# nuclia/nucliadb

Hardware: AMD Instinct MI355X
Metric: queries/sec + recall@10 (768-dim cosine k-NN, HNSW M=30 ef=30 ef_upper=4 build_ef_upper=4, k=10) (higher is better)
Workload: dtype f32

## Files before the change

### include/nidx_gpu.h

```cpp
#ifndef NIDX_GPU_H
#define NIDX_GPU_H

#include <stddef.h>
#include <stdint.h>

#ifdef __cplusplus
extern "C" {
#endif

#define NIDX_OK 0
#define NIDX_ERR_IO (-1)
#define NIDX_ERR_INCONSISTENT_DIMENSIONS (-2)
#define NIDX_ERR_INVALID_CONFIGURATION (-3)
#define NIDX_ERR_EMPTY_MERGE (-4)
#define NIDX_ERR_INVALID_ARGUMENT (-5)
#define NIDX_ERR_UNSUPPORTED (-6)
#define NIDX_ERR_DEVICE (-7)
#define NIDX_ERR_INVALID_GRAPH (-8)
#define NIDX_ERR_INEXACT (-9)
#define NIDX_ERR_OUT_OF_MEMORY (-10)
#define NIDX_ERR_INTERNAL (-11)
#define NIDX_ERR_BUSY (-12)

int32_t nidx_gpu_last_error(char *buf, size_t len);
// ... 244 lines not shown

int32_t nidx_gpu_similarity(const float *x, const float *y, uint32_t n_pairs, uint32_t dimension,
                            int32_t similarity, int32_t order, float *out);
int32_t nidx_gpu_normalize(const float *in, uint32_t n, uint32_t dimension, float *out);

int32_t nidx_gpu_hnsw_graph_check(const uint8_t *graph, uint64_t graph_len, const float *edges, uint64_t n_edges, uint32_t n_nodes,
                                  uint32_t *entry_node_out, uint32_t *entry_layer_out, uint64_t *n_links_out,
                                  uint64_t *n_broken_links_out);

int32_t nidx_gpu_vector_build_hnsw(nidx_gpu_vector_index_t *index, uint32_t segment, uint64_t level_seed);
int32_t nidx_gpu_vector_build_stats(nidx_gpu_vector_index_t *index, uint64_t *stats_out);
int32_t nidx_gpu_vector_extend_hnsw(nidx_gpu_vector_index_t *index, uint32_t segment, uint64_t level_seed);
int32_t nidx_gpu_vector_serialize_hnsw(const nidx_gpu_vector_index_t *index, uint32_t segment, uint8_t *graph_out,
                                       uint64_t graph_cap, uint64_t *graph_len_out, float *edges_out,
                                       uint64_t edges_cap, uint64_t *n_edges_out);

typedef struct nidx_gpu_segment_dir nidx_gpu_segment_dir_t;
int32_t nidx_gpu_segment_dir_open(const char *path, uint32_t dimension, nidx_gpu_segment_dir_t **dir_out);
void nidx_gpu_segment_dir_close(nidx_gpu_segment_dir_t *dir);
int32_t nidx_gpu_segment_dir_index_source(const nidx_gpu_segment_dir_t *dir);
int32_t nidx_gpu_segment_dir_segment(const nidx_gpu_segment_dir_t *dir, nidx_gpu_vector_segment_t *segment_out);
int32_t nidx_gpu_segment_dir_filter_index(const nidx_gpu_segment_dir_t *dir, nidx_gpu_filter_index_t *lists_out);
enum { NIDX_LIST_LABEL = 0, NIDX_LIST_FIELD = 1 };
int32_t nidx_gpu_segment_dir_lists(const nidx_gpu_segment_dir_t *dir, int32_t kind, const uint8_t *key, uint32_t key_len,
                                   int32_t prefix, uint32_t *first_out, uint32_t *count_out);
typedef struct {
    const char *key;
    uint32_t key_len;
    const uint8_t *metadata;
    uint32_t metadata_len;
// ... 615 lines not shown
```

### nucliadb_amd/_lib.py

```python
from __future__ import annotations

import ctypes as C
import os

_HERE = os.path.dirname(os.path.abspath(__file__))
LIB_PATH = os.environ.get("NIDX_GPU_LIB") or os.path.join(_HERE, "libnidx_gpu.so")

NIDX_OK = 0
NIDX_ERR_IO = -1
NIDX_ERR_INCONSISTENT_DIMENSIONS = -2
NIDX_ERR_INVALID_CONFIGURATION = -3
NIDX_ERR_EMPTY_MERGE = -4
NIDX_ERR_INVALID_ARGUMENT = -5
NIDX_ERR_UNSUPPORTED = -6
NIDX_ERR_DEVICE = -7
NIDX_ERR_INVALID_GRAPH = -8
NIDX_ERR_INEXACT = -9
NIDX_ERR_OUT_OF_MEMORY = -10
NIDX_ERR_INTERNAL = -11
NIDX_ERR_BUSY = -12

SIMILARITY_DOT, SIMILARITY_COSINE = 0, 1
METHOD_AUTO, METHOD_HNSW, METHOD_BRUTE_FORCE, METHOD_BRUTE_FORCE_MFMA, METHOD_BRUTE_FORCE_BF16 = 0, 1, 2, 3, 4
METHOD_RABITQ_HNSW, METHOD_RABITQ_BRUTE_FORCE = 5, 6
# ... 430 lines not shown
                                                C.c_void_p, C.c_void_p, C.c_void_p, C.c_void_p]),
    "nidx_gpu_vector_search_maxsim_filtered_per_query": (C.c_int32, [C.c_void_p, C.c_void_p, C.c_void_p, C.c_uint32, C.c_uint32,
                                                                     C.POINTER(VectorSearchParamsC), C.c_void_p, C.c_uint32, C.c_void_p,
                                                                     C.c_void_p, C.c_void_p, C.c_void_p, C.c_void_p]),
    "nidx_gpu_vector_search_maxsim_submit": (C.c_int32, [C.c_void_p, C.c_void_p, C.c_void_p, C.c_uint32, C.c_uint32,
                                                         C.POINTER(VectorSearchParamsC), C.c_void_p, C.POINTER(C.c_uint64)]),
    "nidx_gpu_vector_search_maxsim_submit_filtered_per_query": (C.c_int32, [C.c_void_p, C.c_void_p, C.c_void_p, C.c_uint32, C.c_uint32,
                                                                            C.POINTER(VectorSearchParamsC), C.c_void_p, C.c_uint32,
                                                                            C.c_void_p, C.POINTER(C.c_uint64)]),
    "nidx_gpu_vector_search_maxsim_wait": (C.c_int32, [C.c_void_p, C.c_uint64, C.c_void_p, C.c_void_p, C.c_void_p, C.c_void_p]),
    "nidx_gpu_vector_maxsim_stats": (C.c_int32, [C.c_void_p, C.POINTER(C.c_uint64), C.POINTER(C.c_uint64)]),
    "nidx_gpu_vector_quantize": (C.c_int32, [C.c_void_p, C.c_uint32]),
    "nidx_gpu_vector_serialize_quantized": (C.c_int32, [C.c_void_p, C.c_uint32, C.c_void_p, C.c_uint64, C.POINTER(C.c_uint64)]),
    "nidx_gpu_vector_serialize_hnsw": (C.c_int32, [C.c_void_p, C.c_uint32, C.c_void_p, C.c_uint64, C.POINTER(C.c_uint64),
                                                   C.c_void_p, C.c_uint64, C.POINTER(C.c_uint64)]),
    "nidx_gpu_bm25_open": (C.c_int32, [C.POINTER(Bm25SegmentC), C.c_uint32, C.POINTER(C.c_void_p)]),
    "nidx_gpu_bm25_close": (None, [C.c_void_p]),
    "nidx_gpu_bm25_space_usage": (C.c_int32, [C.c_void_p, C.POINTER(C.c_uint64)]),
    "nidx_gpu_bm25_search": (C.c_int32, [C.c_void_p, C.c_void_p, C.c_void_p, C.c_uint32, C.c_uint32, C.c_void_p, C.c_void_p,
                                         C.c_void_p, C.c_void_p, C.c_void_p, C.c_void_p]),
    "nidx_gpu_bm25_search_ex": (C.c_int32, [C.c_void_p, C.c_void_p, C.c_void_p, C.c_uint32, C.POINTER(Bm25SearchOptionsC), C.c_void_p,
                                          C.c_void_p, C.c_void_p, C.c_void_p, C.c_void_p]),
    "nidx_gpu_bm25_search_submit": (C.c_int32, [C.c_void_p, C.c_void_p, C.c_void_p, C.c_uint32, C.POINTER(Bm25SearchOptionsC), C.POINTER(C.c_uint64)]),
    "nidx_gpu_bm25_search_wait": (C.c_int32, [C.c_void_p, C.c_uint64, C.c_void_p, C.c_void_p, C.c_void_p, C.c_void_p, C.c_void_p]),
    "nidx_gpu_bm25_set_fast_field": (C.c_int32, [C.c_void_p, C.c_uint32, C.c_uint32, C.c_void_p]),
    "nidx_gpu_bm25_set_dictionary": (C.c_int32, [C.c_void_p, C.c_void_p, C.c_void_p]),
    "nidx_gpu_bm25_sync": (C.c_int32, [C.c_void_p, C.POINTER(Bm25SyncEntryC), C.c_uint32, C.c_uint32, C.c_void_p, C.c_void_p, C.c_void_p, C.c_uint32,
                                       C.c_void_p, C.c_void_p, C.POINTER(Bm25SyncStatsC)]),
    "nidx_gpu_bm25_generation": (C.c_int32, [C.c_void_p, C.POINTER(C.c_uint64)]),
    "nidx_gpu_segment_dir_open": (C.c_int32, [C.c_char_p, C.c_uint32, C.POINTER(C.c_void_p)]),
# ... 173 lines not shown
```

### nucliadb_amd/csrc/hnsw_build.hip

```cpp
#include <stdlib.h>

#include <hipcub/hipcub.hpp>

#include "hnsw_device.h"
#include "hnsw_graph.h"

namespace nidx {

struct BuildArgs {
    SegDev seg;
    GraphDev g;
    float *l0_w;
    float *upper_w;
    const uint8_t *levels;
    uint32_t batch_start, batch_size;
    const uint32_t *slot_base;
    uint64_t *found;
    uint32_t *found_len;
    uint32_t *slot_node;
    uint32_t *slot_layer;
    uint64_t *req_key;
    float *req_val;
    uint32_t vis_log2;
    uint32_t ef_upper;
// ... 328 lines not shown
    e = hipcub::DeviceRadixSort::SortPairs(sort_tmp, sort_tmp_bytes, a.req_key, req_key_sorted, a.req_val,
                                           req_val_sorted, (int)n_req, 0, 64, s);
    if (e != hipSuccess) return e;
    if (minw == 4) hipLaunchKernelGGL((reverse_link_kernel<NJ, 4>), dim3((n_req + 3) / 4), dim3(256), 0, s, a, req_key_sorted, req_val_sorted, n_req);
    else if (minw == 2) hipLaunchKernelGGL((reverse_link_kernel<NJ, 2>), dim3((n_req + 3) / 4), dim3(256), 0, s, a, req_key_sorted, req_val_sorted, n_req);
    else hipLaunchKernelGGL((reverse_link_kernel<NJ, 3>), dim3((n_req + 3) / 4), dim3(256), 0, s, a, req_key_sorted, req_val_sorted, n_req);
    return hipGetLastError();
}

__global__ void flag_clear_kernel(uint32_t *word, uint32_t bits) { atomicAnd(word, ~bits); }
hipError_t launch_flag_clear(uint32_t *word, uint32_t bits, hipStream_t s) {
    hipLaunchKernelGGL(flag_clear_kernel, dim3(1), dim3(1), 0, s, word, bits);
    return hipGetLastError();
}

hipError_t build_sort_tmp_bytes(uint32_t max_req, size_t *bytes) {
    *bytes = 0;
    return hipcub::DeviceRadixSort::SortPairs(nullptr, *bytes, (uint64_t *)nullptr, (uint64_t *)nullptr,
                                              (float *)nullptr, (float *)nullptr, (int)max_req, 0, 64, nullptr);
}

hipError_t launch_build_batch(const BuildBatch &b, hipStream_t s) {
    BuildArgs a;
    a.seg = b.seg;
    a.g = b.g;
    a.l0_w = b.l0_w;
    a.upper_w = b.upper_w;
    a.levels = b.levels;
    a.batch_start = b.batch_start;
    a.batch_size = b.batch_size;
// ... 29 lines not shown
```

### nucliadb_amd/csrc/hnsw_build_host.cpp

```cpp
#include <stdlib.h>

#include <algorithm>
#include <chrono>

#include "host_common.h"
#include "vector_index.h"

namespace nidx {

static const uint32_t kMaxBatch = 32768;

int32_t VectorIndex::build_hnsw(uint32_t si, uint64_t level_seed, bool extend) {
    std::lock_guard<std::mutex> lock(mu);
    NIDX_HIP(hipSetDevice(device));
    VectorSegment &seg = segs[si];
    const uint32_t n = seg.n;
    if (extend && !seg.base_graph) return fail(NIDX_ERR_INVALID_ARGUMENT, "segment %u was not opened with a partial hnsw graph", si);
    const uint32_t n0 = extend ? seg.base_nodes : 0;
    const HostGraph *base = extend ? seg.base_graph.get() : nullptr;
    seg.has_graph = false;
    if (n == 0) return NIDX_OK;
    if (n >= (1u << 30)) return fail(NIDX_ERR_UNSUPPORTED, "segments of 2^30 or more vectors are not supported");
    std::vector<uint8_t> drawn, levels(n);
    draw_levels(level_seed, n - n0, drawn);
// ... 179 lines not shown
                d5[1] ? d5[2] / d5[1] : 0, d5[3] ? (double)d5[2] / (double)d5[3] : 0.0);
    }
    if (flags & NIDX_FLAG_POOL_INEXACT) return fail(NIDX_ERR_INEXACT, "HNSW build: candidate pool overflow");
    last_build_flags = flags;
    {
        std::vector<unsigned long long> lines((size_t)NIDX_BUILD_STAT_LINES * 16, 0ull);
        if (b.stats) NIDX_HIP(hipMemcpy(lines.data(), b.stats, lines.size() * 8, hipMemcpyDeviceToHost));
        for (int c = 0; c < 8; c++) last_build_stats[c] = 0;
        for (size_t l = 0; l < NIDX_BUILD_STAT_LINES; l++)
            for (int c = 0; c < 6; c++) last_build_stats[2 + c] += lines[l * 16 + c];
        last_build_stats[0] = n - n0;
        last_build_stats[1] = (uint64_t)std::chrono::duration<double, std::micro>(std::chrono::steady_clock::now() - t_build0).count();
        if (!b.stats) last_build_stats[2] = ~0ull;
    }
    seg.has_graph = true;
    seg.base_graph.reset();
    seg.base_nodes = 0;
    return NIDX_OK;
}

}

using namespace nidx;

extern "C" int32_t nidx_gpu_vector_build_hnsw(nidx_gpu_vector_index_t *index, uint32_t segment, uint64_t level_seed) try {
    VectorIndex *idx = reinterpret_cast<VectorIndex *>(index);
    if (!idx) return fail(NIDX_ERR_INVALID_ARGUMENT, "bad index/segment");
    GenShared gen(idx->gate);
    if (segment >= idx->segs.size()) return fail(NIDX_ERR_INVALID_ARGUMENT, "bad index/segment");
    return idx->build_hnsw(segment, level_seed, false);
// ... 20 lines not shown
```

### nucliadb_amd/csrc/hnsw_device.h

```cpp
#pragma once
#include "device_common.h"
#include "kernels.h"

namespace nidx {

#define NIDX_POOL_CAP 512
#define NIDX_VIS_EMPTY 0xffffffffu
#define NIDX_DEFER_CAP 256

struct NbBuf {
    uint32_t addr[64];
    float ab[64];
    float xx[64];
};
struct SearchShared {
    uint64_t pool[NIDX_POOL_CAP];
    NbBuf nb[2];
    uint32_t eps[256];
    int ctrl[12];
};

template <int NJ>
struct QueryRegs {
    float4 qv[NJ];
// ... 93 lines not shown
        unsigned long long m = __ballot(keep);
        int pos = out + __popcll(m & ((1ull << lane) - 1ull));
        if (keep) pool[pos] = v;
        out += __popcll(m);
    }
    pool_len = out;
}

template <int NL>
struct CandSet {
    uint64_t unexp[NL];
    __device__ inline void init() {
#pragma unroll
        for (int i = 0; i < NL; i++) unexp[i] = 0;
    }
    __device__ inline void insert(WaveTopK<NL> &res, uint64_t nk, int cap, int lane, uint64_t &out_key, bool &out_unexp) {
        uint64_t d = nk, dflag = 1;
#pragma unroll
        for (int i = 0; i < NL; i++) {
            if (d != NIDX_EMPTY_KEY) {
                const int pos = __popcll(__ballot(res.l[i].key > d));
                if (pos < 64) {
                    const uint64_t last = lane_bcast_u64(res.l[i].key, 63);
                    const uint64_t lastflag = unexp[i] >> 63;
                    const uint64_t up = wave_shr1_u64(res.l[i].key);
                    if (lane > pos) res.l[i].key = up;
                    if (lane == pos) res.l[i].key = d;
                    const uint64_t low = unexp[i] & ((1ull << pos) - 1ull);
                    const uint64_t high = pos < 63 ? ((unexp[i] >> pos) << (pos + 1)) : 0ull;
                    unexp[i] = low | (dflag << pos) | high;
                    d = last;
                    dflag = lastflag;
                }
            }
        }
        res.len++;
        out_key = NIDX_EMPTY_KEY;
// ... 158 lines not shown
    for (;;) {
        lds_barrier();
        const int cmd = __builtin_amdgcn_readfirstlane(sh.ctrl[0]);
        const int op = cmd & 3;
        if (op == NIDX_CMD_EVAL) eval_neighbours_dynamic<NJ, EVR>(seg, q, sh.nb[(cmd >> 2) & 1], cmd >> 3, cosine, &sh.ctrl[3]);
        else if (op == NIDX_CMD_CLEAR) vis_clear(vis, vis_cap);
        lds_barrier();
        if (op == NIDX_CMD_EXIT) return;
    }
}

#define NIDX_PARK_SLOTS 4
#define NIDX_EPS_BARE 0
#define NIDX_EPS_PARKED 1
#define NIDX_EPS_CARRIED 2
template <int NJ, int EFL, int EVR, bool SPLIT = false>
__device__ inline void layer_search_block(const SegDev &seg, const GraphDev &g, int layer, int k,
                                          const QueryRegs<NJ> &q, SearchShared &sh, uint32_t *vis, uint32_t vis_log2,
                                          WaveTopK<EFL> &res, SearchCounters &st, int ep_mode = NIDX_EPS_BARE) {
    const int lane = threadIdx.x & 63;
    const bool ctl = SPLIT ? true : (nidx_tid() >> 6) == 0;
    const bool cosine = seg.similarity == 1;
    const uint32_t vis_cap = 1u << vis_log2;
    const bool carried = ep_mode == NIDX_EPS_CARRIED;
    int pool_len = 0;
    uint32_t vis_count = 0;

    if constexpr (SPLIT) {
        split_post(sh, NIDX_CMD_CLEAR, 0, 0, lane);
        vis_clear(vis, vis_cap);
        split_close();
    } else {
        vis_clear(vis, vis_cap);
        __syncthreads();
    }
    int n_new = sh.ctrl[2];
// ... 3 lines not shown
    const int n_eps = carried ? 0 : n_new;
    uint32_t ptag = 0xffffffffu, pbase = 0xffffffffu;
    uint32_t pt0 = 0xffffffffu, pt1 = 0xffffffffu, pt2 = 0xffffffffu, pt3 = 0xffffffffu;
    int n_park = 0;
    if (ep_mode != NIDX_EPS_BARE && n_new <= 64) n_park = n_new < NIDX_PARK_SLOTS ? n_new : NIDX_PARK_SLOTS;
    if (carried && ctl) {
#pragma unroll
        for (int i = 0; i < EFL; i++) {
            const int left = res.len - 64 * i;
            cand.unexp[i] = left >= 64 ? ~0ull : (left > 0 ? (1ull << left) - 1ull : 0ull);
            if (lane < left) vis_insert(vis, vis_log2, rank_key_addr(res.mine(i)));
        }
        st.evals += n_new;
        vis_count += n_new;
        if (lane < n_park) ptag = rank_key_addr(res.mine(0));
    }
    if (ctl && !carried) {
        res.init();
        if (lane < n_new) {
            uint32_t ep = sh.eps[lane];
            vis_insert(vis, vis_log2, ep);
            sh.nb[0].addr[lane] = ep;
            if (lane < n_park) ptag = ep;
        }
    }
    if (layer >= 1 && ptag != 0xffffffffu) pbase = g.upper_base[ptag];
    int ep_done = 0;
    while (ep_done < n_eps) {
        int chunk = n_eps - ep_done < 64 ? n_eps - ep_done : 64;
        if (ctl && ep_done > 0 && lane < chunk) {
            uint32_t ep = sh.eps[ep_done + lane];
            vis_insert(vis, vis_log2, ep);
            sh.nb[0].addr[lane] = ep;
        }
        if constexpr (SPLIT) {
            split_post(sh, NIDX_CMD_EVAL, 0, chunk, lane);
            split_close();
        } else {
            __syncthreads();
            eval_neighbours<NJ, EVR>(seg, q, sh.nb[0], chunk, cosine);
            __syncthreads();
        }
        if (ctl) {
            float s = lane < chunk ? score_from_sums(sh.nb[0].ab[lane], sh.nb[0].xx[lane], q.qq, q.sqrt_qq, cosine) : 0.f;
            uint32_t addr = sh.nb[0].addr[lane];
            for (int j = 0; j < chunk; j++) {
                uint64_t ek;
                bool eu;
                cand.insert(res, rank_key(lane_bcast_f32(s, j), lane_bcast_u32(addr, j)), 64 * EFL, lane, ek, eu);
            }
            st.evals += chunk;
            vis_count += chunk;
        }
        ep_done += chunk;
    }
    if (ctl && n_park > 0) {
        pt0 = lane_bcast_u32(ptag, 0);
        pt1 = lane_bcast_u32(ptag, 1);
        pt2 = lane_bcast_u32(ptag, 2);
        pt3 = lane_bcast_u32(ptag, 3);
        uint32_t w[NIDX_PARK_SLOTS];
#pragma unroll
        for (int r = 0; r < NIDX_PARK_SLOTS; r++) {
            w[r] = 0;
            if (r < n_park) {
                const uint32_t node = lane_bcast_u32(ptag, r), b = lane_bcast_u32(pbase, r);
                if (layer == 0) w[r] = g.l0[(size_t)node * NIDX_L0_STRIDE + lane];
                else if (b != 0xffffffffu && lane < NIDX_UP_STRIDE) w[r] = g.upper[((size_t)b + (layer - 1)) * NIDX_UP_STRIDE + lane];
            }
        }
#pragma unroll
        for (int r = 0; r < NIDX_PARK_SLOTS; r++)
            if (r < n_park) sh.eps[r * 64 + lane] = w[r];
    }

    uint32_t pw0 = 0, pw1 = 0, tg0 = 0xffffffffu, tg1 = 0xffffffffu;
    uint32_t edge_hits = 0;
    auto prepare = [&](uint64_t ck, NbBuf &dst) -> int {
        uint32_t deg;
        const uint32_t node = rank_key_addr(ck);
        uint32_t w;
        const int slot = node == pt0 ? 0 : (node == pt1 ? 1 : (node == pt2 ? 2 : (node == pt3 ? 3 : -1)));
        if (slot >= 0) {
            w = sh.eps[slot * 64 + lane];
            deg = lane_bcast_u32(w, 0);
            edge_hits++;
        } else if (node == tg0) {
            w = pw0;
            deg = lane_bcast_u32(w, 0);
            edge_hits++;
        } else if (node == tg1) {
            w = pw1;
            deg = lane_bcast_u32(w, 0);
            edge_hits++;
        } else {
            w = load_edge_word(g, node, layer, lane, deg);
        }
        const bool fresh = lane >= 1 && lane <= (int)deg && !vis_contains(vis, vis_log2, w);
        const unsigned long long m = __ballot(fresh);
        if (fresh) dst.addr[__popcll(m & ((1ull << lane) - 1ull))] = w;
        return __popcll(m);
    };
    int p = 0;
    uint64_t cur = NIDX_EMPTY_KEY;
    int cont = 0, n_cur_reg = 0;
    if (ctl) {
        const uint64_t t_a = clock64();
        int n0 = 0;
        cur = cand.pop(res);
        if (cur != NIDX_EMPTY_KEY && !(rank_key_score(cur) < res.worst_score())) {
            cont = 1;
            n0 = prepare(cur, sh.nb[0]);
        }
        n_cur_reg = n0;
        if (!SPLIT && lane == 0) {
            sh.ctrl[0] = cont;
            sh.ctrl[6] = n0;
            sh.ctrl[3] = 0;
        }
        st.cyc_ctl += clock64() - t_a;
    }
    if constexpr (SPLIT) {
        if (cont) {
            split_post(sh, NIDX_CMD_EVAL, 0, n_cur_reg, lane);
            split_close();
        }
    } else {
// ... 29 lines not shown
                todo = __ballot(ins);
                const int n_valid = __popcll(todo);
                st.expansions++;
                st.evals += n_valid;
                vis_count += n_valid;
                overflow = vis_count > vis_cap - vis_cap / 4;
                s = ins ? score_from_sums(nb_cur.ab[lane], nb_cur.xx[lane], q.qq, q.sqrt_qq, cosine) : 0.f;
                int n_next = 0;
                if (!overflow) {
                    const float ws = res.worst_score();
                    const bool adm = ins && (s > ws || res.len < k);
                    const uint64_t bn = wave_max_u64(adm ? rank_key(s, addr) : NIDX_EMPTY_KEY);
                    const uint64_t pm = cand.peek(res);
                    nxt = pm > bn ? pm : bn;
                    if (nxt == NIDX_EMPTY_KEY && pool_len > 0) nxt = pool_peek(sh.pool, pool_len, lane);
                    if (nxt != NIDX_EMPTY_KEY) n_next = prepare(nxt, nb_next);
                    if (layer == 0) {
                        uint64_t ka, kb;
                        cand.peek2_except(res, nxt, ka, kb);
                        uint32_t wa = ka != NIDX_EMPTY_KEY ? rank_key_addr(ka) : 0xffffffffu;
                        uint32_t wb = kb != NIDX_EMPTY_KEY ? rank_key_addr(kb) : 0xffffffffu;
                        if (wa == tg1 || wb == tg0) {
                            const uint32_t t = wa;
                            wa = wb;
                            wb = t;
                        }
                        if (wa != tg0) {
                            tg0 = wa;
                            if (wa != 0xffffffffu) pw0 = g.l0[(size_t)wa * NIDX_L0_STRIDE + lane];
                        }
                        if (wb != tg1) {
                            tg1 = wb;
// ... 16 lines not shown
            const int n_next = SPLIT ? n_next_reg : sh.ctrl[6 + (p ^ 1)];
            if (!ctl && has_next) eval_neighbours_dynamic<NJ, EVR>(seg, q, nb_next, n_next, cosine, &sh.ctrl[3]);
            if (ctl) {
                while (todo) {
                    float ws = res.worst_score();
                    if (res.len >= k) {
                        todo &= __ballot(s > ws);
                        if (!todo) break;
                    }
                    int j = __ffsll((long long)todo) - 1;
                    todo &= ~(1ull << j);
                    float sj = lane_bcast_f32(s, j);
                    if (sj > ws || res.len < k) {
                        uint64_t ek;
                        bool eu;
                        cand.insert(res, rank_key(sj, lane_bcast_u32(addr, j)), k, lane, ek, eu);
                        if (eu && ek != NIDX_EMPTY_KEY && !(rank_key_score(ek) < res.worst_score())) {
                            if (pool_len == NIDX_POOL_CAP) {
                                pool_prune(sh.pool, pool_len, res.worst_score(), lane);
                                if (pool_len == NIDX_POOL_CAP) {
                                    st.flags |= NIDX_FLAG_POOL_INEXACT;
                                    pool_len--;
                                }
                            }
                            if (lane == 0) sh.pool[pool_len] = ek;
                            pool_len++;
                        }
                    }
                }
                int redo = 0;
                cont = 0;
// ... 14 lines not shown
                st.cyc_ins += t_c - t_b;
                if (has_next) eval_neighbours_dynamic<NJ, EVR>(seg, q, nb_next, n_next, cosine, &sh.ctrl[3]);
                st.cyc_eval += clock64() - t_c;
            }
            if constexpr (SPLIT) {
                split_close();
            } else {
                lds_barrier();
                cont = sh.ctrl[0];
                redo_reg = sh.ctrl[4];
            }
            if (!cont) break;
            n_cur_reg = n_next;
            if (redo_reg) {
                if (ctl) {
                    const int n1 = prepare(cur, nb_next);
                    n_cur_reg = n1;
                    if (!SPLIT && lane == 0) {
                        sh.ctrl[6 + (p ^ 1)] = n1;
                        sh.ctrl[3] = 0;
                    }
                }
                if constexpr (SPLIT) {
                    split_post(sh, NIDX_CMD_EVAL, p ^ 1, n_cur_reg, lane);
                    split_close();
                } else {
                    lds_barrier();
                    eval_neighbours_dynamic<NJ, EVR>(seg, q, nb_next, sh.ctrl[6 + (p ^ 1)], cosine, &sh.ctrl[3]);
                    lds_barrier();
                }
            }
// ... 9 lines not shown
```

### nucliadb_amd/csrc/hnsw_search.hip

```cpp
#include "hnsw_device.h"

namespace nidx {

template <int NJ>
__device__ inline bool rows_equal(const SegDev &seg, uint32_t a, uint32_t b, int lane) {
    const float *ra = seg.vectors + (size_t)a * seg.dp, *rb = seg.vectors + (size_t)b * seg.dp;
    bool eq = true;
#pragma unroll
    for (int j = 0; j < NJ; j++) {
        uint32_t e = (uint32_t)j * 256u + (uint32_t)lane * 4u;
        if (e < seg.dp) {
            uint4 x = *reinterpret_cast<const uint4 *>(ra + e);
            uint4 y = *reinterpret_cast<const uint4 *>(rb + e);
            eq = eq && x.x == y.x && x.y == y.y && x.z == y.z && x.w == y.w;
        }
    }
    return __all(eq);
}

template <int NJ, int EVR, int EFL, bool SPLIT>
__device__ __forceinline__ void hnsw_search_body(const HnswSearchArgs &a, const uint32_t qi, unsigned char *smem) {
    SearchShared &sh = *reinterpret_cast<SearchShared *>(smem);
    uint32_t *vis = reinterpret_cast<uint32_t *>(smem + sizeof(SearchShared));
    __shared__ uint32_t res_addr[64 * EFL];
// ... 21 lines not shown

    SearchCounters st = {0, 0, 0, 0, 0, 0, 0};
    const uint64_t t_start = clock64();
    WaveTopK<EFL> res;
    res.init();

    if (nidx_tid() == 0) {
        sh.eps[0] = a.g.ep_node;
        sh.ctrl[2] = 1;
    }
    if constexpr (!SPLIT) __syncthreads();
    const bool entry_mode = a.entry_vec != nullptr;
    const int efu = a.ef_upper ? (int)a.ef_upper : 1;
    const int top = entry_mode ? 0 : (int)a.g.ep_layer;
    for (int layer = top; layer >= 1; layer--) {
        layer_search_block<NJ, EFL, EVR, SPLIT>(a.seg, a.g, layer, efu, q, sh, vis, a.vis_log2, res, st, layer == top ? NIDX_EPS_PARKED : NIDX_EPS_CARRIED);
        if (ctl && lane == 0) sh.ctrl[2] = res.len;
    }
    const int efs = a.ef_search ? (int)a.ef_search : NIDX_EF_SEARCH;
    const int ef = k > efs ? k : efs;
    if (!entry_mode) layer_search_block<NJ, EFL, EVR, SPLIT>(a.seg, a.g, 0, ef, q, sh, vis, a.vis_log2, res, st, top >= 1 ? NIDX_EPS_CARRIED : NIDX_EPS_PARKED);
    if (a.dump_vec) {
        if (ctl) {
#pragma unroll
            for (int i = 0; i < EFL; i++) {
                const uint64_t key = res.mine(i);
                const int e = 64 * i + lane;
                if (e < res.len) {
                    a.dump_vec[(size_t)qi * NIDX_DUMP_STRIDE + e] = rank_key_addr(key);
                    a.dump_score[(size_t)qi * NIDX_DUMP_STRIDE + e] = rank_key_score(key);
                }
// ... 446 lines not shown
```

### nucliadb_amd/csrc/kernels.h

```cpp
#pragma once
#define NIDX_K_MAX 512
#include <hip/hip_runtime.h>
#include <stdint.h>

#include "../../include/nidx_gpu.h"
#include "bm25_aux_plan.h"
#include "bm25_work_plan.h"

namespace nidx {

struct ScanArgs {
    const float *vectors;
    const float *norm2;
    uint32_t n, dp;
    const float *queries;
    uint32_t n_queries;
    const uint64_t *alive;
    const uint64_t *filter;
    const uint32_t *para_of_vec;
    int similarity;
    float min_score;
    uint32_t k;
    uint32_t qt;
    uint64_t *partial;
// ... 120 lines not shown

#define NIDX_L0_STRIDE 64
#define NIDX_UP_STRIDE 32
#define NIDX_M 30
#define NIDX_M_MAX 30
#define NIDX_M_MAX0 60
#define NIDX_EF_CONSTRUCTION 100
#define NIDX_EF_SEARCH 30

struct GraphDev {
    uint32_t *l0;
    uint32_t *upper_base;
    uint32_t *upper;
    uint32_t ep_node, ep_layer;
    uint32_t n;
};

struct SegDev {
    const float *vectors;
    const float *norm2;
    uint32_t n, dp, dim;
    const uint32_t *para_of_vec;
    const uint64_t *alive;
    int similarity;
};

#define NIDX_STAT_EVALS 0
#define NIDX_STAT_EXPANSIONS 1
#define NIDX_STAT_VISITED 2
#define NIDX_STAT_FLAGS 3
#define NIDX_STAT_CYC_CTL 4
// ... 536 lines not shown
```

### nucliadb_amd/csrc/vector_index.cpp

```cpp
#include <math.h>
#include <stdio.h>
#include <stdlib.h>
#include <string.h>

#include <algorithm>
#include <unordered_map>
#include <chrono>
#include <map>
#include <memory>
#include <mutex>

#include "device_common.h"
#include "hnsw_graph.h"
#include "host_common.h"
#include "kernels.h"
#include "vector_index.h"
#include "prefilter_handover.h"

namespace nidx {

static thread_local char g_last_error[512];

static void record_error(const char *fmt, va_list ap) { vsnprintf(g_last_error, sizeof(g_last_error), fmt, ap); }

// ... 83 lines not shown
    }
    return c;
}

int32_t VectorSegment::upload_graph(const HostGraph &hg) {
    NIDX_HIP(g_l0.alloc(hg.l0.size() * 4));
    NIDX_HIP(g_upper_base.alloc(hg.upper_base.size() * 4));
    NIDX_HIP(g_upper.alloc(std::max<size_t>(hg.upper.size(), NIDX_UP_STRIDE) * 4));
    NIDX_HIP(hipMemcpy(g_l0.p, hg.l0.data(), hg.l0.size() * 4, hipMemcpyHostToDevice));
    NIDX_HIP(hipMemcpy(g_upper_base.p, hg.upper_base.data(), hg.upper_base.size() * 4, hipMemcpyHostToDevice));
    if (!hg.upper.empty()) NIDX_HIP(hipMemcpy(g_upper.p, hg.upper.data(), hg.upper.size() * 4, hipMemcpyHostToDevice));
    ep_node = hg.ep_node;
    ep_layer = hg.ep_layer;
    top_layer = hg.top_layer;
    has_graph = true;
    return NIDX_OK;
}

GraphDev VectorSegment::graph_dev() const {
    GraphDev g;
    g.l0 = g_l0.as<uint32_t>();
    g.upper_base = g_upper_base.as<uint32_t>();
    g.upper = g_upper.as<uint32_t>();
    g.ep_node = ep_node;
    g.ep_layer = ep_layer;
    g.n = n;
    return g;
}

SegDev VectorSegment::seg_dev(int similarity) const {
    SegDev s;
    s.vectors = vectors.as<float>();
    s.norm2 = norm2.as<float>();
    s.n = n;
    s.dp = dp;
    s.dim = dim;
    s.para_of_vec = identity_para ? nullptr : para_of_vec.as<uint32_t>();
    s.alive = all_alive ? nullptr : alive.as<uint64_t>();
    s.similarity = similarity;
    return s;
}

uint64_t VectorSegment::bytes() const {
    return vectors.bytes + norm2.bytes + norm2_serial.bytes + vectors16.bytes + para_of_vec.bytes + alive.bytes + g_l0.bytes + g_upper_base.bytes +
           g_upper.bytes + g_l0_w.bytes + g_upper_w.bytes + f_offsets.bytes + f_ids.bytes + f_key_bytes.bytes + f_key_offsets.bytes + quant.bytes;
}

static int32_t open_segment(const nidx_gpu_vector_config_t &cfg, const nidx_gpu_vector_segment_t &in, VectorSegment &seg,
                            hipStream_t stream) {
    const uint32_t d = cfg.dimension;
    seg.n = in.n_vectors;
    seg.dim = d;
    seg.dp = (d + 3u) & ~3u;
    seg.n_paragraphs = in.n_paragraphs;
    const uint64_t packed = (uint64_t)d * 4, trailer = packed + 4;
    if (in.n_vectors > 0 && in.vectors == nullptr) return fail(NIDX_ERR_INVALID_ARGUMENT, "segment has no vectors pointer");
    if (in.row_stride_bytes < packed)
        return fail(NIDX_ERR_INCONSISTENT_DIMENSIONS, "Inconsistent dimensions. Index=%u Vector=%llu", d,
                    (unsigned long long)(in.row_stride_bytes / 4));
    std::vector<uint32_t> pov;
// ... 483 lines not shown
    a.out_count = d_out_count;
    a.stats = d_stats;
    a.multi = cfg.vector_cardinality == NIDX_CARDINALITY_MULTI ? 1 : 0;
    a.eval_rows = rows_for(shape_nq);
    a.min_waves = waves_for(shape_nq);
    a.entry_vec = nullptr;
    a.entry_score = nullptr;
    a.entry_count = nullptr;
    a.dump_vec = nullptr;
    a.dump_score = nullptr;
    a.dump_count = nullptr;
    a.flag_word = d_flag_word;
    a.ef_search = ef_search;
    a.ef_upper = ef_upper;
    a.closest_prefetch = closest_prefetch ? 1 : 0;
    a.filter_row = pq_filter_row;
    a.filter_table = pq_filter_table;
    a.filter_words = pq_filter_words;
    return a;
}

ScanArgs VectorIndex::scan_args(uint32_t s, const float *d_queries, uint32_t nq, uint32_t k, float min_score, const uint64_t *d_filter) const {
    const VectorSegment &seg = segs[s];
    ScanArgs a;
    a.vectors = seg.vectors.as<float>();
    a.norm2 = seg.norm2.as<float>();
    a.n = seg.n;
    a.dp = seg.dp;
    a.queries = d_queries;
    a.n_queries = nq;
// ... 1351 lines not shown
    std::string n(name);
    if (n == "waves_per_query") idx->waves_per_query = std::max(1, std::min(4, (int)value));
    else if (n == "eval_rows") { idx->eval_rows = std::max(2, std::min(4, (int)value)); idx->shape_pinned = true; }
    else if (n == "min_waves") { idx->min_waves = value >= 4 ? std::min(6, (int)value) : 2; idx->shape_pinned = true; }
    else if (n == "launch_shape") idx->launch_shape = (int)std::max<int64_t>(0, std::min<int64_t>(2, (int64_t)value));
    else if (n == "vis_log2") { idx->default_vis_log2 = (uint32_t)std::max(10, std::min(15, (int)value)); idx->vis_pinned = true; }
    else if (n == "coalesce_window_us") idx->coalescer_config(value, -1, -1);
    else if (n == "coalesce_max_batch") idx->coalescer_config(-1, value, -1);
    else if (n == "coalesce_in_flight") idx->coalescer_config(-1, -1, value);
    else if (n == "coalesce_max_callers") idx->coalescer_admission(std::max(0, (int)value), -1);
    else if (n == "coalesce_reject_when_full") idx->coalescer_admission(-1, value != 0);
    else if (n == "pipeline_depth") idx->pipeline_config(value);
    else if (n == "pipeline_walks") idx->pipeline_config(-1, value);
    else if (n == "stage_threads") set_stage_threads(value);
    else if (n == "closest_prefetch") idx->closest_prefetch = value != 0;
    else if (n == "per_query_filter_scratch_kib") idx->pq_scratch_cap = value > 0 ? (uint64_t)value << 10 : 1ull << 30;
    else if (n == "serial_segments") idx->serial_segments = value != 0;
    else if (n == "build_vis_log2") { idx->build_vis_log2 = (uint32_t)std::max(10, std::min(15, (int)value)); idx->build_vis_pinned = true; }
    else if (n == "ef_search") {
        if (value < 0 || value > NIDX_K_MAX) return fail(NIDX_ERR_INVALID_ARGUMENT, "ef_search must be in 0..%d", NIDX_K_MAX);
        idx->ef_search = (uint32_t)value;
    }
    else if (n == "build_ef_upper") {
        if (value < 0 || value > 64) return fail(NIDX_ERR_INVALID_ARGUMENT, "build_ef_upper must be in 0..64");
        idx->build_ef_upper = (uint32_t)value;
    }
    else if (n == "ef_upper") {
        if (value < 0 || value > 64) return fail(NIDX_ERR_INVALID_ARGUMENT, "ef_upper must be in 0..64");
        idx->ef_upper = (uint32_t)value;
    }
// ... 381 lines not shown
    std::vector<float> edges;
    serialize_disk_v2(hg, graph, edges);
    if (graph_len_out) *graph_len_out = graph.size();
    if (n_edges_out) *n_edges_out = edges.size();
    if (graph_out) {
        if (graph_cap < graph.size()) return fail(NIDX_ERR_INVALID_ARGUMENT, "graph buffer too small");
        memcpy(graph_out, graph.data(), graph.size());
    }
    if (edges_out) {
        if (edges_cap < edges.size()) return fail(NIDX_ERR_INVALID_ARGUMENT, "edges buffer too small");
        memcpy(edges_out, edges.data(), edges.size() * 4);
    }
    return NIDX_OK;
} NIDX_ABI_CATCH

}
```

### nucliadb_amd/csrc/vector_index.h

```cpp
#pragma once
#include <atomic>
#include <condition_variable>
#include <memory>
#include <mutex>
#include <vector>

#include "filter_stage.h"
#include "hnsw_graph.h"
#include "host_common.h"
#include "kernels.h"

namespace nidx {

bool use_hnsw(uint64_t total_nodes, uint64_t matching_nodes, uint64_t top_k, bool has_rabitq);
void normalize_row(const float *in, float *out, uint32_t d);
void stage_query_rows(const float *src, float *dst, uint32_t nq, uint32_t d, uint32_t dp, bool normalize);
void set_stage_threads(int32_t n);

struct VectorSegment {
    uint32_t n = 0, dim = 0, dp = 0, n_paragraphs = 0;
    DevBuf vectors;
    DevBuf norm2;
    DevBuf norm2_serial;
    DevBuf vectors16;
// ... 5 lines not shown
    bool identity_para = true, all_alive = true;
    std::vector<uint32_t> para_host;
    std::vector<uint32_t> para_first_host, para_num_host;
    std::vector<uint64_t> alive_host;
    uint64_t alive_count = 0;
    std::vector<uint64_t> key_ids;
    DevBuf key_ids_dev;
    DevBuf f_offsets, f_ids;
    DevBuf f_key_bytes, f_key_offsets;
    uint32_t f_n_keys = 0;
    uint32_t f_n_lists = 0;
    uint64_t f_n_ids = 0;
    bool has_graph = false;
    DevBuf g_l0, g_upper_base, g_upper;
    DevBuf g_l0_w, g_upper_w;
    uint32_t ep_node = 0, ep_layer = 0;
    std::vector<uint8_t> top_layer;
    DevBuf quant;
    bool has_quant = false;
    uint32_t base_nodes = 0;
    std::unique_ptr<HostGraph> base_graph;

    int32_t upload_graph(const HostGraph &hg);
    GraphDev graph_dev() const;
    SegDev seg_dev(int similarity) const;
    uint64_t bytes() const;
};

struct GenGate {
    std::mutex mu;
    std::condition_variable cv;
    std::atomic<uint32_t> holders{0};
    std::atomic<bool> pending{false};
    std::atomic<uint64_t> generation{0};
    void enter();
    bool try_enter();
    void enter_nested() { holders.fetch_add(1, std::memory_order_seq_cst); }
    void leave();
// ... 68 lines not shown
    int waves_per_query = 4;
    int eval_rows = 4;
    int min_waves = 4;
    bool shape_pinned = false;
    int rows_for(uint32_t nq) const { return (!shape_pinned && nq <= 256) ? 4 : (shape_pinned && min_waves >= 5) ? 2 : eval_rows; }
    int waves_for(uint32_t nq) const { return (!shape_pinned && nq <= 256) ? 2 : (!shape_pinned && crowded_now()) ? 5 : min_waves; }
    static bool crowded_launch();
    static void set_crowded_launch(bool on);
    int launch_shape = 0;
    bool crowded_now() const { return launch_shape == 1 || (launch_shape == 0 && crowded_launch()); }
    bool vis_pinned = false;
    uint32_t vis_for(uint32_t nq) const { return (!vis_pinned && !shape_pinned && nq > 256 && crowded_now()) ? std::min<uint32_t>(default_vis_log2, 12u) : default_vis_log2; }
    uint32_t ef_search = 0;
    uint32_t ef_upper = 0;
    bool closest_prefetch = true;
    bool serial_segments = false;
    uint32_t default_vis_log2 = 13;
    uint32_t build_vis_log2 = 14;
    bool build_vis_pinned = false;
    uint32_t build_ef_upper = 0;
    uint32_t last_build_flags = 0;
    uint32_t last_build_escalated_at = 0;
    uint64_t last_build_stats[8] = {0, 0, 0, 0, 0, 0, 0, 0};
    DevBuf scratch_fstack, scratch_flists, scratch_fcount, scratch_q16, scratch_cand_vec, scratch_cand_score, scratch_cand_count, scratch_multi_vec, scratch_multi_score, scratch_multi_count, scratch_qnorm, scratch_partial, scratch_queries, scratch_filter, scratch_out_vec, scratch_out_score, scratch_out_count,
        scratch_stats, scratch_rq, scratch_planes, scratch_vis, scratch_ties, scratch_entry_vec, scratch_entry_score, scratch_entry_count,
        scratch_dump_vec, scratch_dump_score, scratch_dump_count, scratch_spill_pool, scratch_spill_cmax, scratch_spill_vis, scratch_spill_ids, scratch_rowmask, scratch_floor, scratch_floor2, scratch_bf16_flags, scratch_bf16_counts;
    uint64_t scan_matching_hint = ~0ull;
    const uint32_t *pq_filter_row = nullptr;
    const uint64_t *pq_filter_table = nullptr;
    uint32_t pq_filter_words = 0;
// ... 131 lines not shown
```

Measured before the change: 4.507 million.

## Precompute upper-layer neighbor slot indices to skip upper_base lookups during search

Builds a parallel array holding, for each upper-layer neighbor edge, that neighbor's base slot in the upper adjacency array. The slots are carried alongside result keys and prefetched edge words during upper-layer search, which avoids a dependent global load of upper_base before fetching each neighbor's edges. It costs extra device memory equal to the upper graph, a build-time kernel, and more LDS/register bookkeeping in the insert path. It only applies to the SPLIT kernel variant and can be turned off with a runtime option.

New measurement: 4.424 million. 0.982x the previous value.

```diff
diff --git a/include/nidx_gpu.h b/include/nidx_gpu.h
--- a/include/nidx_gpu.h
+++ b/include/nidx_gpu.h
@@ -282,6 +282,8 @@
 int32_t nidx_gpu_vector_serialize_hnsw(const nidx_gpu_vector_index_t *index, uint32_t segment, uint8_t *graph_out,
                                        uint64_t graph_cap, uint64_t *graph_len_out, float *edges_out,
                                        uint64_t edges_cap, uint64_t *n_edges_out);
+int32_t nidx_gpu_vector_upper_slots_read(const nidx_gpu_vector_index_t *index, uint32_t segment, uint32_t *slots_out,
+                                         uint64_t cap_words, uint64_t *n_words_out);
 
 typedef struct nidx_gpu_segment_dir nidx_gpu_segment_dir_t;
 int32_t nidx_gpu_segment_dir_open(const char *path, uint32_t dimension, nidx_gpu_segment_dir_t **dir_out);
diff --git a/nucliadb_amd/_lib.py b/nucliadb_amd/_lib.py
--- a/nucliadb_amd/_lib.py
+++ b/nucliadb_amd/_lib.py
@@ -468,6 +468,7 @@
     "nidx_gpu_vector_serialize_quantized": (C.c_int32, [C.c_void_p, C.c_uint32, C.c_void_p, C.c_uint64, C.POINTER(C.c_uint64)]),
     "nidx_gpu_vector_serialize_hnsw": (C.c_int32, [C.c_void_p, C.c_uint32, C.c_void_p, C.c_uint64, C.POINTER(C.c_uint64),
                                                    C.c_void_p, C.c_uint64, C.POINTER(C.c_uint64)]),
+    "nidx_gpu_vector_upper_slots_read": (C.c_int32, [C.c_void_p, C.c_uint32, C.c_void_p, C.c_uint64, C.POINTER(C.c_uint64)]),
     "nidx_gpu_bm25_open": (C.c_int32, [C.POINTER(Bm25SegmentC), C.c_uint32, C.POINTER(C.c_void_p)]),
     "nidx_gpu_bm25_close": (None, [C.c_void_p]),
     "nidx_gpu_bm25_space_usage": (C.c_int32, [C.c_void_p, C.POINTER(C.c_uint64)]),
diff --git a/nucliadb_amd/csrc/hnsw_build.hip b/nucliadb_amd/csrc/hnsw_build.hip
--- a/nucliadb_amd/csrc/hnsw_build.hip
+++ b/nucliadb_amd/csrc/hnsw_build.hip
@@ -366,6 +366,26 @@
     return hipGetLastError();
 }
 
+__global__ __launch_bounds__(256) void upper_slots_kernel(const uint32_t *__restrict__ upper, const uint32_t *__restrict__ upper_base, uint32_t n,
+                                                          uint32_t n_upper, uint32_t *__restrict__ slots) {
+    const size_t i = (size_t)blockIdx.x * 256 + threadIdx.x;
+    if (i >= (size_t)n_upper * NIDX_UP_STRIDE) return;
+    const uint32_t j = (uint32_t)(i % NIDX_UP_STRIDE);
+    const uint32_t deg = upper[i - j];
+    uint32_t v = 0xffffffffu;
+    if (j >= 1 && j <= deg) {
+        const uint32_t nb = upper[i];
+        if (nb < n) v = upper_base[nb];
+    }
+    slots[i] = v;
+}
+hipError_t launch_upper_slots(const uint32_t *upper, const uint32_t *upper_base, uint32_t n, uint32_t n_upper, uint32_t *slots, hipStream_t s) {
+    if (n_upper == 0) return hipSuccess;
+    const size_t words = (size_t)n_upper * NIDX_UP_STRIDE;
+    hipLaunchKernelGGL(upper_slots_kernel, dim3((unsigned)((words + 255) / 256)), dim3(256), 0, s, upper, upper_base, n, n_upper, slots);
+    return hipGetLastError();
+}
+
 hipError_t build_sort_tmp_bytes(uint32_t max_req, size_t *bytes) {
     *bytes = 0;
     return hipcub::DeviceRadixSort::SortPairs(nullptr, *bytes, (uint64_t *)nullptr, (uint64_t *)nullptr,
diff --git a/nucliadb_amd/csrc/hnsw_build_host.cpp b/nucliadb_amd/csrc/hnsw_build_host.cpp
--- a/nucliadb_amd/csrc/hnsw_build_host.cpp
+++ b/nucliadb_amd/csrc/hnsw_build_host.cpp
@@ -217,6 +217,11 @@
         if (!b.stats) last_build_stats[2] = ~0ull;
     }
     seg.has_graph = true;
+    {
+        const int32_t r = seg.build_upper_slots(stream);
+        if (r != NIDX_OK) return r;
+        NIDX_HIP(hipStreamSynchronize(stream));
+    }
     seg.base_graph.reset();
     seg.base_nodes = 0;
     return NIDX_OK;
diff --git a/nucliadb_amd/csrc/hnsw_device.h b/nucliadb_amd/csrc/hnsw_device.h
--- a/nucliadb_amd/csrc/hnsw_device.h
+++ b/nucliadb_amd/csrc/hnsw_device.h
@@ -131,13 +131,23 @@
 #pragma unroll
         for (int i = 0; i < NL; i++) unexp[i] = 0;
     }
-    __device__ inline void insert(WaveTopK<NL> &res, uint64_t nk, int cap, int lane, uint64_t &out_key, bool &out_unexp) {
+    template <bool S = false>
+    __device__ inline void insert(WaveTopK<NL> &res, uint64_t nk, int cap, int lane, uint64_t &out_key, bool &out_unexp, uint32_t *rslot = nullptr,
+                                  uint32_t nslot = 0xffffffffu) {
         uint64_t d = nk, dflag = 1;
 #pragma unroll
         for (int i = 0; i < NL; i++) {
             if (d != NIDX_EMPTY_KEY) {
                 const int pos = __popcll(__ballot(res.l[i].key > d));
                 if (pos < 64) {
+                    if constexpr (S) {
+                        if (i == 0) {
+                            const bool mv = lane >= pos && lane < 63;
+                            const uint32_t up_s = mv ? rslot[lane] : 0u;
+                            if (mv) rslot[lane + 1] = up_s;
+                            if (lane == pos) rslot[lane] = nslot;
+                        }
+                    }
                     const uint64_t last = lane_bcast_u64(res.l[i].key, 63);
                     const uint64_t lastflag = unexp[i] >> 63;
                     const uint64_t up = wave_shr1_u64(res.l[i].key);
@@ -326,12 +336,14 @@
 #define NIDX_EPS_BARE 0
 #define NIDX_EPS_PARKED 1
 #define NIDX_EPS_CARRIED 2
-template <int NJ, int EFL, int EVR, bool SPLIT = false>
+template <int NJ, int EFL, int EVR, bool SPLIT = false, bool SLOTS = false>
 __device__ inline void layer_search_block(const SegDev &seg, const GraphDev &g, int layer, int k,
                                           const QueryRegs<NJ> &q, SearchShared &sh, uint32_t *vis, uint32_t vis_log2,
-                                          WaveTopK<EFL> &res, SearchCounters &st, int ep_mode = NIDX_EPS_BARE) {
+                                          WaveTopK<EFL> &res, SearchCounters &st, int ep_mode = NIDX_EPS_BARE,
+                                          uint32_t *rslot = nullptr, uint32_t *slot_lds = nullptr) {
     const int lane = threadIdx.x & 63;
     const bool ctl = SPLIT ? true : (nidx_tid() >> 6) == 0;
+    const bool slots_on = SLOTS && g.upper_slots != nullptr;
     const bool cosine = seg.similarity == 1;
     const uint32_t vis_cap = 1u << vis_log2;
     const bool carried = ep_mode == NIDX_EPS_CARRIED;
@@ -365,9 +377,12 @@
         st.evals += n_new;
         vis_count += n_new;
         if (lane < n_park) ptag = rank_key_addr(res.mine(0));
+        if constexpr (SLOTS)
+            if (lane < n_park) pbase = rslot[lane];
     }
     if (ctl && !carried) {
         res.init();
+        if constexpr (SLOTS) rslot[lane] = 0xffffffffu;
         if (lane < n_new) {
             uint32_t ep = sh.eps[lane];
             vis_insert(vis, vis_log2, ep);
@@ -375,7 +390,7 @@
             if (lane < n_park) ptag = ep;
         }
     }
-    if (layer >= 1 && ptag != 0xffffffffu) pbase = g.upper_base[ptag];
+    if (layer >= 1 && ptag != 0xffffffffu && pbase == 0xffffffffu) pbase = g.upper_base[ptag];
     int ep_done = 0;
     while (ep_done < n_eps) {
         int chunk = n_eps - ep_done < 64 ? n_eps - ep_done : 64;
@@ -398,7 +413,7 @@
             for (int j = 0; j < chunk; j++) {
                 uint64_t ek;
                 bool eu;
-                cand.insert(res, rank_key(lane_bcast_f32(s, j), lane_bcast_u32(addr, j)), 64 * EFL, lane, ek, eu);
+                cand.template insert<SLOTS>(res, rank_key(lane_bcast_f32(s, j), lane_bcast_u32(addr, j)), 64 * EFL, lane, ek, eu, rslot);
             }
             st.evals += chunk;
             vis_count += chunk;
@@ -418,6 +433,10 @@
                 const uint32_t node = lane_bcast_u32(ptag, r), b = lane_bcast_u32(pbase, r);
                 if (layer == 0) w[r] = g.l0[(size_t)node * NIDX_L0_STRIDE + lane];
                 else if (b != 0xffffffffu && lane < NIDX_UP_STRIDE) w[r] = g.upper[((size_t)b + (layer - 1)) * NIDX_UP_STRIDE + lane];
+                if constexpr (SLOTS) {
+                    if (lane >= NIDX_UP_STRIDE)
+                        w[r] = slots_on && b != 0xffffffffu ? g.upper_slots[((size_t)b + (layer - 1)) * NIDX_UP_STRIDE + (lane - NIDX_UP_STRIDE)] : 0xffffffffu;
+                }
             }
         }
 #pragma unroll
@@ -427,13 +446,15 @@
 
     uint32_t pw0 = 0, pw1 = 0, tg0 = 0xffffffffu, tg1 = 0xffffffffu;
     uint32_t edge_hits = 0;
-    auto prepare = [&](uint64_t ck, NbBuf &dst) -> int {
+    auto prepare = [&](uint64_t ck, int b, uint32_t ks) -> int {
+        NbBuf &dst = sh.nb[b];
         uint32_t deg;
         const uint32_t node = rank_key_addr(ck);
-        uint32_t w;
+        uint32_t w, sw = 0xffffffffu;
         const int slot = node == pt0 ? 0 : (node == pt1 ? 1 : (node == pt2 ? 2 : (node == pt3 ? 3 : -1)));
         if (slot >= 0) {
             w = sh.eps[slot * 64 + lane];
+            if constexpr (SLOTS) sw = sh.eps[slot * 64 + NIDX_UP_STRIDE + (lane & (NIDX_UP_STRIDE - 1))];
             deg = lane_bcast_u32(w, 0);
             edge_hits++;
         } else if (node == tg0) {
@@ -444,13 +465,34 @@
             w = pw1;
             deg = lane_bcast_u32(w, 0);
             edge_hits++;
+        } else if constexpr (SLOTS) {
+            uint32_t base = ks;
+            if (base == 0xffffffffu) base = g.upper_base[node];
+            else edge_hits++;
+            w = 0;
+            if (base != 0xffffffffu && lane < NIDX_UP_STRIDE) {
+                const size_t at = ((size_t)base + (layer - 1)) * NIDX_UP_STRIDE + lane;
+                w = g.upper[at];
+                if (slots_on) sw = g.upper_slots[at];
+            }
+            deg = lane_bcast_u32(w, 0);
         } else {
             w = load_edge_word(g, node, layer, lane, deg);
         }
         const bool fresh = lane >= 1 && lane <= (int)deg && !vis_contains(vis, vis_log2, w);
         const unsigned long long m = __ballot(fresh);
-        if (fresh) dst.addr[__popcll(m & ((1ull << lane) - 1ull))] = w;
+        const int pos = __popcll(m & ((1ull << lane) - 1ull));
+        if (fresh) dst.addr[pos] = w;
+        if constexpr (SLOTS)
+            if (fresh && pos < NIDX_UP_STRIDE) slot_lds[NIDX_UP_STRIDE * b + pos] = sw;
         return __popcll(m);
+    };
+    auto slot_of = [&](uint64_t key) -> uint32_t {
+        if constexpr (SLOTS) {
+            const unsigned long long mm = __ballot(res.l[0].key == key);
+            if (mm) return (uint32_t)__builtin_amdgcn_readfirstlane((int)rslot[__builtin_ctzll(mm)]);
+        }
+        return 0xffffffffu;
     };
     int p = 0;
     uint64_t cur = NIDX_EMPTY_KEY;
@@ -461,7 +503,7 @@
         cur = cand.pop(res);
         if (cur != NIDX_EMPTY_KEY && !(rank_key_score(cur) < res.worst_score())) {
             cont = 1;
-            n0 = prepare(cur, sh.nb[0]);
+            n0 = prepare(cur, 0, slot_of(cur));
         }
         n_cur_reg = n0;
         if (!SPLIT && lane == 0) {
@@ -521,8 +563,15 @@
                     const uint64_t pm = cand.peek(res);
                     nxt = pm > bn ? pm : bn;
                     if (nxt == NIDX_EMPTY_KEY && pool_len > 0) nxt = pool_peek(sh.pool, pool_len, lane);
-                    if (nxt != NIDX_EMPTY_KEY) n_next = prepare(nxt, nb_next);
-                    if (layer == 0) {
+                    if (nxt != NIDX_EMPTY_KEY) {
+                        uint32_t ks = slot_of(nxt);
+                        if constexpr (SLOTS) {
+                            const unsigned long long mm = __ballot(adm && rank_key(s, addr) == nxt) & 0xffffffffull;
+                            if (ks == 0xffffffffu && mm) ks = (uint32_t)__builtin_amdgcn_readfirstlane((int)slot_lds[NIDX_UP_STRIDE * p + __builtin_ctzll(mm)]);
+                        }
+                        n_next = prepare(nxt, p ^ 1, ks);
+                    }
+                    if (!SLOTS && layer == 0) {
                         uint64_t ka, kb;
                         cand.peek2_except(res, nxt, ka, kb);
                         uint32_t wa = ka != NIDX_EMPTY_KEY ? rank_key_addr(ka) : 0xffffffffu;
@@ -569,7 +618,10 @@
                     if (sj > ws || res.len < k) {
                         uint64_t ek;
                         bool eu;
-                        cand.insert(res, rank_key(sj, lane_bcast_u32(addr, j)), k, lane, ek, eu);
+                        uint32_t sj_slot = 0xffffffffu;
+                        if constexpr (SLOTS)
+                            if (j < NIDX_UP_STRIDE) sj_slot = (uint32_t)__builtin_amdgcn_readfirstlane((int)slot_lds[NIDX_UP_STRIDE * p + j]);
+                        cand.template insert<SLOTS>(res, rank_key(sj, lane_bcast_u32(addr, j)), k, lane, ek, eu, rslot, sj_slot);
                         if (eu && ek != NIDX_EMPTY_KEY && !(rank_key_score(ek) < res.worst_score())) {
                             if (pool_len == NIDX_POOL_CAP) {
                                 pool_prune(sh.pool, pool_len, res.worst_score(), lane);
@@ -614,7 +666,7 @@
             n_cur_reg = n_next;
             if (redo_reg) {
                 if (ctl) {
-                    const int n1 = prepare(cur, nb_next);
+                    const int n1 = prepare(cur, p ^ 1, slot_of(cur));
                     n_cur_reg = n1;
                     if (!SPLIT && lane == 0) {
                         sh.ctrl[6 + (p ^ 1)] = n1;
diff --git a/nucliadb_amd/csrc/hnsw_search.hip b/nucliadb_amd/csrc/hnsw_search.hip
--- a/nucliadb_amd/csrc/hnsw_search.hip
+++ b/nucliadb_amd/csrc/hnsw_search.hip
@@ -59,7 +59,8 @@
     const int efu = a.ef_upper ? (int)a.ef_upper : 1;
     const int top = entry_mode ? 0 : (int)a.g.ep_layer;
     for (int layer = top; layer >= 1; layer--) {
-        layer_search_block<NJ, EFL, EVR, SPLIT>(a.seg, a.g, layer, efu, q, sh, vis, a.vis_log2, res, st, layer == top ? NIDX_EPS_PARKED : NIDX_EPS_CARRIED);
+        layer_search_block<NJ, EFL, EVR, SPLIT, SPLIT>(a.seg, a.g, layer, efu, q, sh, vis, a.vis_log2, res, st,
+                                                       layer == top ? NIDX_EPS_PARKED : NIDX_EPS_CARRIED, res_addr, res_para);
         if (ctl && lane == 0) sh.ctrl[2] = res.len;
     }
     const int efs = a.ef_search ? (int)a.ef_search : NIDX_EF_SEARCH;
diff --git a/nucliadb_amd/csrc/kernels.h b/nucliadb_amd/csrc/kernels.h
--- a/nucliadb_amd/csrc/kernels.h
+++ b/nucliadb_amd/csrc/kernels.h
@@ -158,7 +158,9 @@
     uint32_t *upper;
     uint32_t ep_node, ep_layer;
     uint32_t n;
-};
+    const uint32_t *upper_slots = nullptr;
+};
+hipError_t launch_upper_slots(const uint32_t *upper, const uint32_t *upper_base, uint32_t n, uint32_t n_upper, uint32_t *slots, hipStream_t s);
 
 struct SegDev {
     const float *vectors;
diff --git a/nucliadb_amd/csrc/vector_index.cpp b/nucliadb_amd/csrc/vector_index.cpp
--- a/nucliadb_amd/csrc/vector_index.cpp
+++ b/nucliadb_amd/csrc/vector_index.cpp
@@ -121,6 +121,16 @@
     ep_layer = hg.ep_layer;
     top_layer = hg.top_layer;
     has_graph = true;
+    int32_t r = build_upper_slots(nullptr);
+    if (r != NIDX_OK) return r;
+    NIDX_HIP(hipStreamSynchronize(nullptr));
+    return NIDX_OK;
+}
+
+int32_t VectorSegment::build_upper_slots(hipStream_t stream) {
+    const size_t n_upper = g_upper.bytes / ((size_t)NIDX_UP_STRIDE * 4);
+    NIDX_HIP(g_upper_slots.alloc(g_upper.bytes));
+    NIDX_HIP(launch_upper_slots(g_upper.as<uint32_t>(), g_upper_base.as<uint32_t>(), n, (uint32_t)n_upper, g_upper_slots.as<uint32_t>(), stream));
     return NIDX_OK;
 }
 
@@ -129,6 +139,7 @@
     g.l0 = g_l0.as<uint32_t>();
     g.upper_base = g_upper_base.as<uint32_t>();
     g.upper = g_upper.as<uint32_t>();
+    g.upper_slots = has_graph ? g_upper_slots.as<uint32_t>() : nullptr;
     g.ep_node = ep_node;
     g.ep_layer = ep_layer;
     g.n = n;
@@ -150,7 +161,7 @@
 
 uint64_t VectorSegment::bytes() const {
     return vectors.bytes + norm2.bytes + norm2_serial.bytes + vectors16.bytes + para_of_vec.bytes + alive.bytes + g_l0.bytes + g_upper_base.bytes +
-           g_upper.bytes + g_l0_w.bytes + g_upper_w.bytes + f_offsets.bytes + f_ids.bytes + f_key_bytes.bytes + f_key_offsets.bytes + quant.bytes;
+           g_upper.bytes + g_upper_slots.bytes + g_l0_w.bytes + g_upper_w.bytes + f_offsets.bytes + f_ids.bytes + f_key_bytes.bytes + f_key_offsets.bytes + quant.bytes;
 }
 
 static int32_t open_segment(const nidx_gpu_vector_config_t &cfg, const nidx_gpu_vector_segment_t &in, VectorSegment &seg,
@@ -664,6 +675,7 @@
     a.ef_search = ef_search;
     a.ef_upper = ef_upper;
     a.closest_prefetch = closest_prefetch ? 1 : 0;
+    if (!upper_slots) a.g.upper_slots = nullptr;
     a.filter_row = pq_filter_row;
     a.filter_table = pq_filter_table;
     a.filter_words = pq_filter_words;
@@ -2045,6 +2057,7 @@
     else if (n == "pipeline_walks") idx->pipeline_config(-1, value);
     else if (n == "stage_threads") set_stage_threads(value);
     else if (n == "closest_prefetch") idx->closest_prefetch = value != 0;
+    else if (n == "upper_slots") idx->upper_slots = value != 0;
     else if (n == "per_query_filter_scratch_kib") idx->pq_scratch_cap = value > 0 ? (uint64_t)value << 10 : 1ull << 30;
     else if (n == "serial_segments") idx->serial_segments = value != 0;
     else if (n == "build_vis_log2") { idx->build_vis_log2 = (uint32_t)std::max(10, std::min(15, (int)value)); idx->build_vis_pinned = true; }
@@ -2456,4 +2469,24 @@
     return NIDX_OK;
 } NIDX_ABI_CATCH
 
-}
+int32_t nidx_gpu_vector_upper_slots_read(const nidx_gpu_vector_index_t *index, uint32_t segment, uint32_t *slots_out, uint64_t cap_words,
+                                         uint64_t *n_words_out) try {
+    const VectorIndex *idx = reinterpret_cast<const VectorIndex *>(index);
+    if (!idx) return fail(NIDX_ERR_INVALID_ARGUMENT, "bad index/segment");
+    GenShared gen(idx->gate);
+    if (segment >= idx->segs.size()) return fail(NIDX_ERR_INVALID_ARGUMENT, "bad index/segment");
+    const VectorSegment &seg = idx->segs[segment];
+    if (!seg.has_graph) return fail(NIDX_ERR_INVALID_ARGUMENT, "segment has no HNSW graph");
+    uint64_t n_upper = 0;
+    for (uint32_t i = 0; i < seg.n; i++) n_upper += seg.top_layer[i];
+    const uint64_t words = n_upper * NIDX_UP_STRIDE;
+    if (n_words_out) *n_words_out = words;
+    if (slots_out) {
+        if (cap_words < words || seg.g_upper_slots.bytes < words * 4) return fail(NIDX_ERR_INVALID_ARGUMENT, "slot buffer too small");
+        NIDX_HIP(hipSetDevice(idx->device));
+        if (words) NIDX_HIP(hipMemcpy(slots_out, seg.g_upper_slots.p, words * 4, hipMemcpyDeviceToHost));
+    }
+    return NIDX_OK;
+} NIDX_ABI_CATCH
+
+}
diff --git a/nucliadb_amd/csrc/vector_index.h b/nucliadb_amd/csrc/vector_index.h
--- a/nucliadb_amd/csrc/vector_index.h
+++ b/nucliadb_amd/csrc/vector_index.h
@@ -43,6 +43,7 @@
     bool has_graph = false;
     DevBuf g_l0, g_upper_base, g_upper;
     DevBuf g_l0_w, g_upper_w;
+    DevBuf g_upper_slots;
     uint32_t ep_node = 0, ep_layer = 0;
     std::vector<uint8_t> top_layer;
     DevBuf quant;
@@ -51,6 +52,7 @@
     std::unique_ptr<HostGraph> base_graph;
 
     int32_t upload_graph(const HostGraph &hg);
+    int32_t build_upper_slots(hipStream_t stream);
     GraphDev graph_dev() const;
     SegDev seg_dev(int similarity) const;
     uint64_t bytes() const;
@@ -149,6 +151,7 @@
     uint32_t ef_search = 0;
     uint32_t ef_upper = 0;
     bool closest_prefetch = true;
+    bool upper_slots = true;
     bool serial_segments = false;
     uint32_t default_vis_log2 = 13;
     uint32_t build_vis_log2 = 14;
```
